# LunaJang/Metabuli_work

Measured on AMD Instinct MI355X. Metric: reads/sec classified (150bp & 10kb) vs GTDB-scale DB at 1/2/4/8 MI355X, higher is better.
Workload: dtype u64

## Files before the change

include/mtb_gpu.h:

```cpp
#ifndef MTB_GPU_H
#define MTB_GPU_H

#include <stddef.h>
#include <stdint.h>

#ifdef __cplusplus
extern "C" {
#endif

#define MTB_OK 0
#define MTB_RETRY 1
#define MTB_ERR_ARG (-1)
#define MTB_ERR_IO (-2)
#define MTB_ERR_HIP (-3)
#define MTB_ERR_DB (-4)
#define MTB_ERR_OOM (-5)
#define MTB_ERR_UNSUPPORTED (-6)
#define MTB_ERR_INTERNAL (-7)

#define MTB_INPUT_DEVICE 1u
#define MTB_KEEP_STAGES 2u
#define MTB_MATCH_ONLY 4u

typedef struct mtb_params {
// ... 77 lines not shown
                      mtb_ctx** out);
void mtb_close(mtb_ctx* ctx);
const char* mtb_last_error(void);
int mtb_set_stream(mtb_ctx* ctx, void* hip_stream);
uint64_t mtb_db_kmers(const mtb_ctx* ctx);
uint64_t mtb_workspace_bytes(const mtb_ctx* ctx);
int mtb_open_phases(const mtb_ctx* ctx, double* sec, int n);
int mtb_set_workspace_cap(mtb_ctx* ctx, uint64_t bytes);
int mtb_release_workspace(mtb_ctx* ctx);
int mtb_ctx_device(const mtb_ctx* ctx);

int mtb_classify_batch(mtb_ctx* ctx, const char* seq, const uint64_t* off, const char* seq2,
                       const uint64_t* off2, uint32_t n_reads, uint32_t flags, mtb_result* results);
int mtb_get_taxcnt(mtb_ctx* ctx, mtb_taxcnt* out, uint64_t capacity, uint64_t* n_out);
int mtb_device_results(mtb_ctx* ctx, void** results, void** taxcnt, uint64_t* n_taxcnt);
int mtb_last_counts(const mtb_ctx* ctx, uint64_t* query_kmers, uint64_t* matches);
int mtb_last_stats(const mtb_ctx* ctx, uint64_t* out, int n);
int mtb_last_stage_ms(const mtb_ctx* ctx, float* ms, int n);
int mtb_last_kernel_ms(const mtb_ctx* ctx, float* ms, int n);
int mtb_copy_results(mtb_ctx* ctx, void* dst, int dst_on_device);
int mtb_copy_taxcnt(mtb_ctx* ctx, void* dst, int dst_on_device, uint64_t* n_out);

int mtb_get_query_kmers(mtb_ctx* ctx, mtb_kmer* out, uint64_t capacity, uint64_t* n_out);
int mtb_get_matches(mtb_ctx* ctx, mtb_match* out, uint64_t capacity, uint64_t* n_out);
int mtb_assign_matches(mtb_ctx* ctx, const mtb_match* matches, uint64_t n_matches,
                       const uint32_t* query_len, uint32_t n_reads, mtb_result* results);

int mtb_mask_reads(mtb_ctx* ctx, const char* seq, const uint64_t* off, uint32_t n_reads, char* out);

int mtb_memcpy(void* dst, const void* src, uint64_t bytes);

int mtb_hamming(int device, const uint64_t* query, const uint64_t* target, uint64_t n, uint8_t* sum, uint16_t* fwd,
                uint16_t* rev);

#define MTB_PIN_SCORE_INCREMENT 0
#define MTB_PIN_HAMMING_INCREMENT 1
#define MTB_PIN_IS_CONSECUTIVE 2
#define MTB_PIN_IS_CONSECUTIVE2 3
#define MTB_PIN_MATCH_SCORE 4
#define MTB_PIN_RIGHT_PART_SCORE 5
#define MTB_PIN_LEFT_PART_SCORE 6
#define MTB_PIN_RIGHT_PART_HAMMING 7
#define MTB_PIN_LEFT_PART_HAMMING 8
#define MTB_PIN_MAX_COVERED_LENGTH 9
#define MTB_PIN_QUERY_KMER_NUMBER 10
#define MTB_PIN_TAXONOMER_SHAPE 11
// ... 150 lines not shown
```

metabuli_work_amd/_lib.py:

```python
import ctypes
import pathlib

from ._abi import MtbClassifyOpts, MtbClassifyStats, MtbDbHost, MtbDbResident, MtbEmStats, MtbParams, MtbReadBatch

_HERE = pathlib.Path(__file__).resolve().parent
LIB_PATH = _HERE / "libmtbgpu.so"
_LIB = None

EXPORTED = [
    "mtb_default_params", "mtb_load_db_parameters", "mtb_open", "mtb_open_host", "mtb_close", "mtb_last_error",
    "mtb_set_stream", "mtb_db_kmers", "mtb_classify_batch", "mtb_get_taxcnt", "mtb_device_results",
    "mtb_clone", "mtb_last_counts", "mtb_last_stats", "mtb_last_stage_ms", "mtb_last_kernel_ms", "mtb_copy_results", "mtb_get_query_kmers",
    "mtb_get_matches", "mtb_assign_matches", "mtb_build_db", "mtb_free_built", "mtb_reader_open", "mtb_reader_next",
    "mtb_reader_close", "mtb_taxon_rank", "mtb_write_classifications", "mtb_partition_bounds", "mtb_copy_matches",
    "mtb_assign_chunks", "mtb_open_resident", "mtb_write_report", "mtb_copy_taxcnt", "mtb_original_taxid",
    "mtb_taxon_lineage", "mtb_start_classify", "mtb_get_em_mappings", "mtb_em", "mtb_write_em_results",
    "mtb_ctx_device", "mtb_start_classify_multi", "mtb_mask_reads", "mtb_workspace_bytes", "mtb_set_workspace_cap",
    "mtb_open_phases", "mtb_start_classify_partitioned", "mtb_release_workspace", "mtb_hamming", "mtb_memcpy",
    "mtb_line_ext_check", "mtb_link_check", "mtb_pin_eval", "mtb_sort_pairs",
    "mtb_merge_db", "mtb_merge_db_dirs", "mtb_merge_last_ms", "mtb_merge_tile_items",
]


class MtbError(RuntimeError):
    pass


def lib() -> ctypes.CDLL:
    global _LIB
    if _LIB is not None:
        return _LIB
    if not LIB_PATH.exists():
        raise MtbError(f"{LIB_PATH} not built: the HIP extension is required (no CPU fallback)")
    L = ctypes.CDLL(str(LIB_PATH))
    vp, u32, u64, i32 = ctypes.c_void_p, ctypes.c_uint32, ctypes.c_uint64, ctypes.c_int
    P = ctypes.POINTER
    L.mtb_default_params.argtypes = [P(MtbParams)]
    L.mtb_default_params.restype = None
    L.mtb_load_db_parameters.argtypes = [ctypes.c_char_p, P(MtbParams)]
    L.mtb_open.argtypes = [ctypes.c_char_p, P(MtbParams), i32, P(vp)]
    L.mtb_open_host.argtypes = [P(MtbDbHost), P(MtbParams), i32, P(vp)]
    L.mtb_open_resident.argtypes = [P(MtbDbResident), P(MtbDbHost), P(MtbParams), i32, P(vp)]
    L.mtb_close.argtypes = [vp]
    L.mtb_clone.argtypes = [vp, P(vp)]
    L.mtb_close.restype = None
    L.mtb_last_error.restype = ctypes.c_char_p
    L.mtb_set_stream.argtypes = [vp, vp]
    L.mtb_db_kmers.argtypes = [vp]
    L.mtb_db_kmers.restype = u64
    L.mtb_workspace_bytes.argtypes = [vp]
    L.mtb_workspace_bytes.restype = u64
    L.mtb_set_workspace_cap.argtypes = [vp, u64]
    L.mtb_release_workspace.argtypes = [vp]
    L.mtb_open_phases.argtypes = [vp, P(ctypes.c_double), i32]
    L.mtb_classify_batch.argtypes = [vp, vp, vp, vp, vp, u32, u32, vp]
    L.mtb_get_taxcnt.argtypes = [vp, vp, u64, P(u64)]
    L.mtb_device_results.argtypes = [vp, P(vp), P(vp), P(u64)]
    L.mtb_last_counts.argtypes = [vp, P(u64), P(u64)]
    L.mtb_last_stats.argtypes = [vp, P(u64), i32]
    L.mtb_last_stage_ms.argtypes = [vp, P(ctypes.c_float), i32]
    L.mtb_last_kernel_ms.argtypes = [vp, P(ctypes.c_float), i32]
    L.mtb_copy_results.argtypes = [vp, vp, i32]
    L.mtb_copy_taxcnt.argtypes = [vp, vp, i32, P(u64)]
    L.mtb_get_query_kmers.argtypes = [vp, vp, u64, P(u64)]
    L.mtb_get_matches.argtypes = [vp, vp, u64, P(u64)]
    L.mtb_assign_matches.argtypes = [vp, vp, u64, vp, u32, vp]
    L.mtb_partition_bounds.argtypes = [vp, u64, u64, i32, vp, vp]
    L.mtb_copy_matches.argtypes = [vp, vp, vp, vp, i32]
    L.mtb_assign_chunks.argtypes = [vp, vp, u64, vp, u32, vp, u32, u32, vp]
    L.mtb_reader_open.argtypes = [ctypes.c_char_p, ctypes.c_char_p, P(vp)]
    L.mtb_reader_next.argtypes = [vp, u32, u64, P(MtbReadBatch)]
    L.mtb_reader_close.argtypes = [vp]
    L.mtb_reader_close.restype = None
    L.mtb_taxon_rank.argtypes = [vp, ctypes.c_int32]
    L.mtb_taxon_rank.restype = ctypes.c_char_p
    L.mtb_write_classifications.argtypes = [vp, ctypes.c_char_p, i32, P(MtbReadBatch), vp, vp, u32]
    L.mtb_original_taxid.argtypes = [vp, ctypes.c_int32]
    L.mtb_original_taxid.restype = ctypes.c_int32
    L.mtb_taxon_lineage.argtypes = [vp, ctypes.c_int32]
    L.mtb_taxon_lineage.restype = ctypes.c_char_p
    L.mtb_start_classify.argtypes = [vp, P(MtbClassifyOpts), P(MtbClassifyStats)]
    L.mtb_start_classify_multi.argtypes = [P(vp), i32, P(MtbClassifyOpts), P(MtbClassifyStats)]
    L.mtb_start_classify_partitioned.argtypes = [P(vp), i32, P(MtbClassifyOpts), P(MtbClassifyStats)]
    L.mtb_ctx_device.argtypes = [vp]
    L.mtb_mask_reads.argtypes = [vp, vp, vp, u32, vp]
    L.mtb_hamming.argtypes = [i32, vp, vp, u64, vp, vp, vp]
    L.mtb_pin_eval.argtypes = [i32, i32, vp, vp, vp, u64, vp, vp]
    L.mtb_sort_pairs.argtypes = [i32, vp, vp, u64, i32, i32, vp, vp]
# ... 22 lines not shown
```

metabuli_work_amd/csrc/mtb_api.hip:

```cpp
#include <chrono>
#include <cmath>
#include <cstdio>
#include <cstring>
#include <string>
#include <vector>
#include <algorithm>
#include <memory>
#include <charconv>
#include <mutex>
#include <unordered_map>

#include "mtb_host.h"
#include "mtb_launch.h"
#include <cstdlib>

using namespace mtb;

#define HIP_TRY(x)                                                                                   \
    do {                                                                                             \
        hipError_t e_ = (x);                                                                         \
        if (e_ != hipSuccess) {                                                                      \
            set_error(std::string("HIP error ") + hipGetErrorString(e_) + " at " #x);                 \
            return e_ == hipErrorOutOfMemory ? MTB_ERR_OOM : MTB_ERR_HIP;                            \
        }                                                                                            \
// ... 91 lines not shown
    uint64_t rankLo = 0, rankHi = ~0ull;
    int joinMode = 0;
    uint64_t* tileRec = nullptr;
    uint32_t* tilePre = nullptr;
    uint64_t nTiles = 0;
    uint32_t sweepNom = 2048;
    uint32_t sweepLdsCap = ~0u;
    bool sweepSmall = false;
    bool filterThreadMajor = false;
    int sweepPersist = 1;
    uint32_t matchWinCap = ~0u;
    bool directJoin = true;
    bool directRetry = false;
    int pruneAfter = 2;
    int bigGroups = 1;
    bool fuseFilter = true;
    bool radixDigits = true;
    bool radixAtomicFirst = false;
    int binnedSort = 0;
    uint64_t binRcForce = 0;
    bool binDigits = true;
    bool uniformUnits = true;
    uint32_t upr = 0;
    uint64_t binHost[kSortBins] = {};
    bool noFilter = false;
    uint32_t spillShift = 0;
    bool sparse = false;
    uint32_t maxW = 0;
    int sortLoFine = kQuerySortLoFine;
    bool forceGeneric = false;
    bool segsortGlobal = false;
    uint32_t mergeSeg = 0;
    int waveTaxon = -1;
    int emulateAll = 0;
    bool pruneCompact = true;
    bool noAlias = false;
    uint64_t aliasBytes = 0;
    int32_t* spOf = nullptr;
    int32_t maxTax = 0;
    int32_t *tNodeOf = nullptr, *tNodeTax = nullptr, *tParent = nullptr, *tDepth = nullptr, *tSpParent = nullptr;
    uint8_t* tFlags = nullptr;
    uint32_t cladePerMatch = 2;
    std::vector<int32_t> hNodeOf;
    std::vector<std::string> hRank;
    HostTaxonomy hTax;
    mutable std::vector<std::string> lineage;
// ... 251 lines not shown
    if (const char* e = getenv("MTB_K6_ALIAS")) c->noAlias = atoi(e) == 0;
    if (c->forceGeneric) c->matchWinCap = 0;
    c->dir = make_aa_dir(c->D, par->kmer_format);
    HIP_TRY(hipMalloc(&c->dirMem, (c->dir.R + 1) * sizeof(uint64_t)));
    c->dir.dir = c->dirMem;
    build_aa_dir(c->db, c->D, c->dir, c->dirMem, s);
    HIP_TRY(hipStreamSynchronize(s));
    c->openS[2] = since(tp);
    if (const char* e = getenv("MTB_JOIN"))
        c->joinMode = !strcmp(e, "sort") ? 1 : !strcmp(e, "probe") ? 2 : !strcmp(e, "sweep") ? 3 : 0;
    if (const char* e = getenv("MTB_SWEEP_NOM")) c->sweepNom = std::max(64u, std::min(4096u, (uint32_t)atoi(e)));
    if (const char* e = getenv("MTB_SWEEP_LDS")) c->sweepLdsCap = (uint32_t)strtoul(e, nullptr, 10);
    if (const char* e = getenv("MTB_SWEEP_PERSIST")) c->sweepPersist = std::max(0, std::min(2, atoi(e)));
    if (const char* e = getenv("MTB_SWEEP_SMALL")) c->sweepSmall = atoi(e) != 0;
    if (const char* e = getenv("MTB_FILTER_PACK")) c->filterThreadMajor = std::string(e) == "thread";
    if ((c->sweepSmall || c->sweepPersist == 2) && !getenv("MTB_SWEEP_NOM")) c->sweepNom = 1024;
    if (const char* e = getenv("MTB_FILTER")) c->noFilter = atoi(e) == 0;
    if (const char* e = getenv("MTB_RADIX_DIGITS")) c->radixDigits = atoi(e) != 0;
    if (const char* e = getenv("MTB_RADIX_ATOMIC_FIRST")) c->radixAtomicFirst = atoi(e) != 0;
    if (const char* e = getenv("MTB_K1F_BINS")) c->binnedSort = atoi(e);
    if (const char* e = getenv("MTB_K1F_BINS_RC")) c->binRcForce = strtoull(e, nullptr, 10);
    if (const char* e = getenv("MTB_K1F_BINS_DIG")) c->binDigits = atoi(e) != 0;
    if (const char* e = getenv("MTB_UNIFORM_UNITS")) c->uniformUnits = atoi(e) != 0;
    if (!c->forceGeneric && !(c->joinMode == 3 && c->noFilter)) {
        HIP_TRY(hipMalloc(&c->lines, kProbeLines * sizeof(ProbeLine)));
        HIP_TRY(hipMemsetAsync(c->lines, 0, kProbeLines * sizeof(ProbeLine), s));
        build_probe_lines(c->db, c->D, c->dir, c->lines, s);
        const char* ll = getenv("MTB_LINK_LINES");
        if ((!ll || atoi(ll) != 0) && c->joinMode != 2 && c->joinMode != 3) {
            if (hipMalloc(&c->link, kLinkSlots * sizeof(uint64_t)) == hipSuccess) {
                build_link_lines(c->lines, c->link, s);
            } else {
                (void)hipGetLastError();
                c->link = nullptr;
            }
        }
        HIP_TRY(hipStreamSynchronize(s));
        c->openS[3] = since(tp);
        const char* ri = getenv("MTB_RUN_INDEX");
        if ((!ri || atoi(ri) != 0) && c->joinMode != 3) {
            uint32_t* pop = nullptr;
            void* tmp = nullptr;
            uint64_t P = 0;
            HIP_TRY(hipMalloc(&c->lineP, (kProbeLines + 1) * sizeof(uint64_t)));
            HIP_TRY(hipMalloc(&pop, kProbeLines * sizeof(uint32_t)));
            HIP_TRY(hipMalloc(&tmp, scan_tmp_elems(kProbeLines) * sizeof(uint64_t)));
// ... 176 lines not shown
    c->matchWinCap = src->matchWinCap;
    c->directJoin = src->directJoin;
    c->directRetry = src->directRetry;
    c->pruneAfter = src->pruneAfter;
    c->bigGroups = src->bigGroups;
    c->fuseFilter = src->fuseFilter;
    c->presentShare = src->presentShare;
    c->spillShift = src->spillShift;
    c->sortLoFine = src->sortLoFine;
    c->forceGeneric = src->forceGeneric;
    c->segsortGlobal = src->segsortGlobal;
    c->mergeSeg = src->mergeSeg;
    c->waveTaxon = src->waveTaxon;
    c->emulateAll = src->emulateAll;
    c->pruneCompact = src->pruneCompact;
    c->noAlias = src->noAlias;
    c->noFilter = src->noFilter;
    c->radixDigits = src->radixDigits;
    c->radixAtomicFirst = src->radixAtomicFirst;
    c->binnedSort = src->binnedSort;
    c->binRcForce = src->binRcForce;
    c->binDigits = src->binDigits;
    c->uniformUnits = src->uniformUnits;
    bind_workspace(c, src->ws.cap);
    *out = c;
    return MTB_OK;
}

#define MTB_BATCH_BUFS(X) \
    X(seq1) X(off1) X(seq2) X(off2) X(meta) X(reserve) X(slotOff) X(qlen) X(scanTmp) X(keysA) X(valsA) X(keysB) \
    X(valsB) X(radixCounts) X(radixOffs) X(readCnt) X(mOff) X(matches) X(matchesSorted) X(segScratch) X(maxSeg) \
    X(errFlag) X(ordKA) X(ordVA) X(ordKB) X(ordVB) X(matchWin) X(unitRead) X(unitInfo) X(waveList) X(waveCount) \
    X(devStats) X(mStage) X(mRank) X(mDirect) X(ovFlag) X(mTotal) X(qFrom) X(probeStats) X(longList) X(longCnt) \
    X(qStart) X(chunkIn) X(chunkCnt) X(chunkSrcOff) X(liveCnt) X(liveOff) X(segLen) X(sizeLists) X(digA) \
    X(digB) X(binCnt) X(binTab) X(local) X(paths) X(comb) X(conn) X(spScore) X(spKeep) X(runFlag) X(runCnt) \
    X(runScan) X(pathCnt) X(gStart) X(sStart) X(runGroup) X(clade) X(tcPool) X(tcLen) X(tcOff) X(tcOut) X(results) \
    X(emMap) X(emCnt) X(emScratch) X(emPacked) X(emCnt32) X(emOff) X(maskOut1) X(maskOut2) X(maskProb) \
    X(maskScale) X(readLens) X(readCnt64)
static std::vector<DevBuf*> batch_bufs(mtb_ctx* c) {
#define MTB_BUF_PTR(n) &c->n,
    return {MTB_BATCH_BUFS(MTB_BUF_PTR)};
#undef MTB_BUF_PTR
}

static const char* const* batch_buf_names() {
#define MTB_BUF_NAME(n) #n,
// ... 325 lines not shown
            HIP_TRY(hipGetLastError());
            if (R) c->presentShare = std::max(c->presentShare, std::min(1.0, 1.125 * (double)Q / (double)R));
            bool over = false;
            for (int r = 0; r < kSortBins; r++) over |= c->binHost[r] > rc;
            if (!over) {
                binRc = rc;
                break;
            }
            c->stats[15]++;
            cap = std::min<uint64_t>(R, Q + Q / 8);
            binned = false;
        }
        for (int pass = 0; pass < 2 && !binRc; pass++) {
            HIP_TRY(c->keysB.ensure(8 * cap));
            HIP_TRY(c->valsB.ensure(4 * cap));
            if (digits) HIP_TRY(c->digA.ensure(cap));
            cap = std::min<uint64_t>(c->keysB.bytes / 8, c->valsB.bytes / 4);
            if (digits) cap = std::min<uint64_t>(cap, c->digA.bytes);
            Q = launch_extract_filter(dSeq1, dOff1, dSeq2, dOff2, c->meta.as<ReadMeta>(), c->slotOff.as<uint64_t>(),
                                      c->unitRead.as<uint32_t>(), U, C, c->tables, c->par.kmer_format, c->par.syncmer,
                                      c->par.smer_len, c->unitInfo.as<uint64_t>(), c->lines, c->keysB.as<uint64_t>(),
                                      c->valsB.as<uint32_t>(), c->mTotal.as<unsigned long long>(), c->rankLo,
                                      c->rankHi, &c->Qall, cap, c->filterThreadMajor, s,
                                      digits ? c->digA.as<uint8_t>() : nullptr, nullptr, 0, nullptr, c->upr, c->link);
            HIP_TRY(hipGetLastError());
            if (Q == ~0ull) {
                set_error("internal error: K1F sequence stage overflow");
                return MTB_ERR_INTERNAL;
            }
            if (R) c->presentShare = std::max(c->presentShare, std::min(1.0, 1.125 * (double)Q / (double)R));
            if (Q <= cap) break;
            cap = std::min<uint64_t>(R, Q + Q / 8);
            c->stats[15]++;
        }
        HIP_TRY(c->keysA.ensure(8 * std::max<uint64_t>(Q, 1)));
        HIP_TRY(c->valsA.ensure(4 * std::max<uint64_t>(Q, 1)));
        if (digits) HIP_TRY(c->digB.ensure(std::max<uint64_t>(Q, 16)));
        qk = c->keysB.as<uint64_t>();
        qi = c->valsB.as<uint32_t>();
    } else if (filt) {
        if (probe) HIP_TRY(c->qFrom.ensure(8 * Rc + 8 * kDbPad));
        Q = launch_filter(c->keysA.as<uint64_t>(), R, c->lines, c->keysB.as<uint64_t>(), c->valsB.as<uint32_t>(),
                          probe ? c->qFrom.as<uint64_t>() : nullptr, c->mTotal.as<unsigned long long>(), c->rankLo,
                          c->rankHi, &c->Qall, s);
        qk = c->keysB.as<uint64_t>();
        qi = c->valsB.as<uint32_t>();
        qf = c->qFrom.as<uint64_t>();
// ... 946 lines not shown
    }
    if (nTop > cap) return MTB_RETRY;
    uint64_t w = 0;
    for (uint32_t i = 0; i < S; i++) {
        if (!isTop[i]) continue;
        if (sp_ids) sp_ids[w] = spTax[i];
        if (sp_probs) sp_probs[w] = p[i];
        if (sp_counts) sp_counts[w] = (unsigned int)(p[i] * (double)qc);
        w++;
    }
    return MTB_OK;
}

int mtb_copy_taxcnt(mtb_ctx* c, void* dst, int dst_on_device, uint64_t* n_out) {
    if (!c || (!dst && c->nTaxcnt)) return MTB_ERR_ARG;
    if (n_out) *n_out = c->nTaxcnt;
    if (c->nTaxcnt)
        HIP_TRY(hipMemcpyAsync(dst, c->tcOut.p, sizeof(mtb_taxcnt) * c->nTaxcnt,
                               dst_on_device ? hipMemcpyDeviceToDevice : hipMemcpyDeviceToHost, c->stream));
    HIP_TRY(hipStreamSynchronize(c->stream));
    return MTB_OK;
}

int mtb_get_query_kmers(mtb_ctx* c, mtb_kmer* out, uint64_t cap, uint64_t* n_out) {
    if (!c || !n_out) return MTB_ERR_ARG;
    *n_out = c->Q;
    if (!c->keepStages) { set_error("batch was not run with MTB_KEEP_STAGES"); return MTB_ERR_ARG; }
    if (c->probed) { set_error("the probe join keeps no sorted query k-mers (MTB_JOIN=probe)"); return MTB_ERR_ARG; }
    if (!c->qSlots) { set_error("no query k-mers kept"); return MTB_ERR_ARG; }
    if (cap < c->Q) return MTB_RETRY;
    std::vector<uint64_t> k(c->Q), ui((c->unitInfo.bytes + 7) / 8);
    std::vector<uint32_t> v(c->Q);
    const void* kp = c->qKeys;
    const void* vp = c->qSlots;
    if (c->Q) {
        HIP_TRY(hipMemcpy(k.data(), kp, 8 * c->Q, hipMemcpyDeviceToHost));
        HIP_TRY(hipMemcpy(v.data(), vp, 4 * c->Q, hipMemcpyDeviceToHost));
        HIP_TRY(hipMemcpy(ui.data(), c->unitInfo.p, c->unitInfo.bytes, hipMemcpyDeviceToHost));
    }
    const bool packed = c->par.kmer_format == 2;
    for (uint64_t i = 0; i < c->Q; i++)
        out[i] = mtb_kmer{packed ? host_from_rank_form(k[i]) : k[i], slot_info(v[i], c->chunkC, ui.data(),
                                                                               c->par.kmer_format)};
    return MTB_OK;
}

// ... 209 lines not shown
```

metabuli_work_amd/csrc/mtb_kernels.hip:

```cpp
#include "mtb_launch.h"

#include <cstring>

namespace mtb {

constexpr int kBlock = 256;
constexpr int kWaves = kBlock / 64;

__device__ __forceinline__ unsigned long long wave_inclusive_scan(unsigned long long x) {
    const int lane = threadIdx.x & 63;
#pragma unroll
    for (int d = 1; d < 64; d <<= 1) {
        unsigned long long y = __shfl_up(x, d, 64);
        if (lane >= d) x += y;
    }
    return x;
}

__device__ __forceinline__ unsigned long long block_exclusive_scan(unsigned long long x, unsigned long long* total) {
    __shared__ unsigned long long wsum[kWaves];
    const int lane = threadIdx.x & 63, w = threadIdx.x >> 6;
    unsigned long long inc = wave_inclusive_scan(x);
    if (lane == 63) wsum[w] = inc;
    __syncthreads();
// ... 185 lines not shown
};

struct UnitWindows {
    const uint8_t* seq;
    int s0, e0;
    int pFirst, nWin;
    bool fromLeft, comp;
    uint64_t info0;
    uint64_t stretch;
};

__device__ __forceinline__ UnitWindows unit_windows(uint64_t u, uint64_t nUnits, uint32_t C,
                                                    const uint8_t* __restrict__ seq1, const uint64_t* __restrict__ off1,
                                                    const uint8_t* __restrict__ seq2, const uint64_t* __restrict__ off2,
                                                    const ReadMeta* __restrict__ meta, const uint64_t* __restrict__ uOff,
                                                    const uint32_t* __restrict__ unitRead, int kmerFormat,
                                                    uint32_t upr) {
    UnitWindows w{};
    if (u >= nUnits) return w;
    const uint32_t r = upr ? (uint32_t)(u / upr) : unitRead[u];
    const ReadMeta m = meta[r];
    const uint64_t first = upr ? (uint64_t)r * upr : uOff[r];
    w.stretch = first | (upr ? (uint64_t)upr : uOff[r + 1] - first) << 40;
    uint32_t local = (uint32_t)(u - first);
    const uint32_t c1 = upr ? 1u : (uint32_t)(m.w1 + C - 1) / C, c2 = upr ? 1u : (uint32_t)(m.w2 + C - 1) / C;
    uint32_t cpf = c1;
    int mate = 0;
    if (local >= 6 * c1) { local -= 6 * c1; mate = 1; cpf = c2; }
    const int frame = (int)(local / cpf);
    const int chunk = (int)(local % cpf);
    const int W = mate ? m.w2 : m.w1;
    w.pFirst = chunk * (int)C;
    w.nWin = min((int)C, W - w.pFirst);
    if (w.nWin <= 0) return w;
    w.seq = mate ? seq2 + off2[r] : seq1 + off1[r];
    const int len = mate ? m.len2 : m.len1;
    const int used = mate ? m.ql2 : m.ql1;
    const uint32_t posOffset = mate ? (uint32_t)m.ql1 + 3u : 0u;
    const bool fwd = frame < 3;
    int begin;
    if (fwd) begin = frame;
    else { begin = (len % 3) - (frame % 3); if (begin < 0) begin += 3; }
    w.s0 = begin;
    w.e0 = begin + used - 1;
    w.fromLeft = (kmerFormat == 2) ? fwd : !fwd;
    w.comp = !fwd;
    const uint32_t pos0 = w.fromLeft ? (uint32_t)(w.s0 + 3 * w.pFirst) : (uint32_t)(w.e0 - 3 * (w.pFirst + 8) + 1);
    w.info0 = pack_info(r + 1, pos0 + posOffset, (uint32_t)frame);
    return w;
}

struct WinScanner {
    const UnitWindows& w;
    const uint8_t* seq;
    const uint8_t* sBase;
    const int8_t *sAA, *sNum;
    int syncmer, nSm;
    uint64_t smMask;
    uint64_t aaAcc = 0, dnaAcc = 0, smAcc = 0;
    uint64_t sm0 = 0, sm1 = 0, sm2 = 0, sm3 = 0, sm4 = 0, sm5 = 0, sm6 = 0, sm7 = 0;
    int run = 0, j;
    uint32_t first7 = 0, firstAA = 0, lastAA = 0;

    __device__ __forceinline__ WinScanner(const UnitWindows& w_, const uint8_t* b, const int8_t* a, const int8_t* n,
                                          int sync, int smerLen, const uint8_t* seqAt)
        : w(w_), seq(seqAt), sBase(b), sAA(a), sNum(n), syncmer(sync), nSm(8 - smerLen + 1),
          smMask((smerLen >= 13) ? ~0ull : ((1ull << (5 * smerLen)) - 1)), j(w_.pFirst) {
        if (w.nWin > 0)
            for (int k = 0; k < 7; k++) codon();
    }
    __device__ __forceinline__ void codon() {
// ... 2193 lines not shown
    }
    unsigned long long tot;
    const unsigned long long off =
        block_exclusive_scan((unsigned long long)__popc(mask) | ((unsigned long long)emitted << 32), &tot) &
        0xFFFFFFFFull;
    if (threadIdx.x == 0) {
        const unsigned long long present = tot & 0xFFFFFFFFull;
        sBase = present ? atomicAdd(counter, present) : 0;
        if (tot >> 32) atomicAdd(counter + 1, tot >> 32);
    }
    __syncthreads();
    uint64_t pos = sBase + off;
#pragma unroll
    for (int j = 0; j < kFilterPer; j++) {
        if (!((mask >> j) & 1u)) continue;
        qkey[pos] = k[j];
        qslot[pos] = (uint32_t)(base + 256ull * j);
        if (FROM) qfrom[pos] = line_lower_bound(lines, k[j] >> 24);
        pos++;
    }
}

constexpr uint32_t kBinStage = 2560;
constexpr uint32_t kSeqStage = 10240;
template <int kPer, bool kJMajor, bool kBinned = false, int kLink = 0, bool kSplit = false, bool kSeqLds = false,
          bool kWavePack = false>
__global__ void __launch_bounds__(256) __attribute__((amdgpu_waves_per_eu(kLink == 4 ? 4 : 1))) k_extract_filter(const uint8_t* __restrict__ seq1, const uint64_t* __restrict__ off1,
                                                        const uint8_t* __restrict__ seq2, const uint64_t* __restrict__ off2,
                                                        const ReadMeta* __restrict__ meta, const uint64_t* __restrict__ uOff,
                                                        const uint32_t* __restrict__ unitRead, uint64_t nUnits, uint32_t C,
                                                        ExtractTables tabs, int kmerFormat, int syncmer, int smerLen,
                                                        uint64_t* __restrict__ unitInfo, const ProbeLine* __restrict__ lines,
                                                        uint64_t* __restrict__ qkey, uint32_t* __restrict__ qslot,
                                                        unsigned long long* __restrict__ counter, uint64_t rankLo,
                                                        uint64_t rankHi, uint64_t cap, uint8_t* __restrict__ qdig,
                                                        unsigned long long* __restrict__ binCnt, uint64_t binRc,
                                                        uint32_t upr, const uint64_t* __restrict__ link,
                                                        int emitPerBlock = 0) {
    static_assert(kLink == 0 || kPer % 2 == 0, "windows probed in pairs");
    __shared__ uint8_t sBase[256];
    __shared__ uint32_t sBin[256];
    __shared__ uint32_t sBinBase[256];
    extern __shared__ uint64_t sStageKey[];
    __shared__ int8_t sAA[64], sNum[64];
    __shared__ unsigned long long sOut;
    __shared__ uint32_t sMaxWin, sCnt[kPer * kWaves], sEx[kWaves][64];
    const int lane = (int)(threadIdx.x & 63), wv = (int)(threadIdx.x >> 6);
    const unsigned long long ltMask = (1ull << lane) - 1;
    if (threadIdx.x == 0) sMaxWin = 0;
    load_extract_tables(tabs, sBase, sAA, sNum);
    const uint64_t u = (uint64_t)blockIdx.x * blockDim.x + threadIdx.x;
    const uint64_t slotBase = (u >> 6) * 64ull * C + (u & 63u);
    const UnitWindows w = unit_windows(u, nUnits, C, seq1, off1, seq2, off2, meta, uOff, unitRead, kmerFormat, upr);
    if (w.nWin > 0) {
        reinterpret_cast<ulonglong2*>(unitInfo)[u] = make_ulonglong2(w.info0, w.stretch);
        atomicMax(&sMaxWin, (uint32_t)w.nWin);
    }
    __shared__ uint8_t sSeq[kSeqLds ? kSeqStage : 1];
    const uint8_t* seqAt = kSeqLds ? sSeq : w.seq;
    if constexpr (kSeqLds) {
        const uint64_t u0 = (uint64_t)blockIdx.x * blockDim.x, uL = min(u0 + blockDim.x, nUnits) - 1;
        const uint64_t r0 = u0 / upr, r1 = uL / upr;
        const uint64_t a1 = off1[r0], n1 = off1[r1 + 1] - a1;
        const uint64_t a2 = seq2 ? off2[r0] : 0, n2 = seq2 ? off2[r1 + 1] - a2 : 0;
        if (n1 + n2 <= kSeqStage) {
            for (uint32_t i = threadIdx.x; i < n1; i += blockDim.x) sSeq[i] = seq1[a1 + i];
            for (uint32_t i = threadIdx.x; i < n2; i += blockDim.x) sSeq[n1 + i] = seq2[a2 + i];
            if (w.nWin > 0) {
                const uint64_t r = u / upr;
                seqAt = (u - r * upr) >= 6u ? sSeq + n1 + (off2[r] - a2) : sSeq + (off1[r] - a1);
            }
        } else if (threadIdx.x == 0) {
            atomicOr(counter + 1, 1ull << 63);
        }
    }
    __syncthreads();
    WinScanner sc(w, sBase, sAA, sNum, syncmer, smerLen, seqAt);
    __syncthreads();
    const uint32_t gEnd = min(C, sMaxWin);
    uint32_t emitted = 0;
    for (uint32_t g = 0; g < gEnd; g += kPer) {
        const uint32_t* const src = kLink ? reinterpret_cast<const uint32_t*>(link) : reinterpret_cast<const uint32_t*>(lines);
        uint64_t k[kPer];
        uint32_t word[kPer], sh[kPer];
        uint32_t f0 = 0, t0 = 0, h0 = 0, y0 = 0;
        bool ok0 = false;
#pragma unroll
        for (int j = 0; j < kPer; j++) {
            k[j] = (int)(g + j) < w.nWin ? sc.next() : kSentinel;
            if constexpr (kLink) {
                const uint64_t r = k[j] >> 24;
                const bool ok = k[j] != kSentinel && r >= rankLo && r < rankHi;
                const uint32_t h = sc.first7, y = sc.lastAA, f = sc.firstAA;
                if (!(j & 1)) {
                    f0 = f, h0 = h, y0 = y, ok0 = ok;
                    t0 = (uint32_t)(r - (uint64_t)f * kLinkSlots);
                    continue;
                }
                const bool shared = ok0 && ok && t0 == h;
                word[j - 1] = !ok0 ? 0u : (shared ? 2u * t0 + 1u : 2u * h0);
                word[j] = !ok ? 0u : 2u * h;
                sh[j - 1] = !ok0 ? 32u : (shared ? f0 : y0);
                sh[j] = !ok ? 32u : y;
                if constexpr (!kSplit) {
                    word[j - 1] = src[word[j - 1]];
                    word[j] = src[word[j]];
                }
            } else {
                word[j] = 0;
                sh[j] = 32;
                const uint64_t xr = k[j] >> 24;
                if (k[j] != kSentinel && xr >= rankLo && xr < rankHi) {
// ... 146 lines not shown
    for (int d = 32; d > 0; d >>= 1) emitted += (uint32_t)__shfl_xor((int)emitted, d, 64);
    if (emitPerBlock) {
        __shared__ uint32_t sEmit[kWaves];
        if ((threadIdx.x & 63) == 0) sEmit[wv] = emitted;
        __syncthreads();
        if (threadIdx.x == 0) {
            uint32_t e = 0;
#pragma unroll
            for (int i = 0; i < kWaves; i++) e += sEmit[i];
            if (e) atomicAdd(counter + 1, (unsigned long long)e);
        }
        return;
    }
    if ((threadIdx.x & 63) == 0 && emitted) atomicAdd(counter + 1, (unsigned long long)emitted);
}

uint64_t launch_extract_filter(const uint8_t* seq1, const uint64_t* off1, const uint8_t* seq2, const uint64_t* off2,
                               const ReadMeta* meta, const uint64_t* uOff, const uint32_t* unitRead, uint64_t nUnits,
                               uint32_t C, const HostTables& t, int kmerFormat, int syncmer, int smerLen,
                               uint64_t* unitInfo, const ProbeLine* lines, uint64_t* qkey, uint32_t* qslot,
                               unsigned long long* counter, uint64_t rankLo, uint64_t rankHi, uint64_t* emitted,
                               uint64_t cap, bool threadMajor, hipStream_t s, uint8_t* qdig,
                               unsigned long long* binCnt, uint64_t binRc, uint64_t* binHost, uint32_t upr,
                               const uint64_t* link) {
    if (binRc) {
        threadMajor = false;
        hipMemsetAsync(binCnt, 0, kSortBins * sizeof(unsigned long long), s);
    }
    hipMemsetAsync(counter, 0, 2 * sizeof(unsigned long long), s);
    if (nUnits) {
        const uint64_t threads = (nUnits + 63) / 64 * 64;
        static const int per = getenv("MTB_FILTER_PER") && atoi(getenv("MTB_FILTER_PER")) == 8 ? 8 : 16;
        const bool jMajor = !threadMajor;
        const unsigned blocks = (unsigned)((threads + 255) / 256);
        const size_t lds = binRc ? kBinStage * (sizeof(uint64_t) + sizeof(uint32_t)) : 0;
#define MTB_EF(P, J)                                                                                                  \
    k_extract_filter<P, J, false, 0, true><<<blocks, 256, lds, s>>>(seq1, off1, seq2, off2, meta, uOff, unitRead, nUnits, C, \
                                                  extract_tables(t), kmerFormat, syncmer, smerLen, unitInfo, lines, qkey, \
                                                  qslot, counter, rankLo, rankHi, cap, qdig, binCnt, binRc, upr, nullptr)
        if (binRc) {
            k_extract_filter<kFilterPer, true, true><<<blocks, 256, lds, s>>>(
                seq1, off1, seq2, off2, meta, uOff, unitRead, nUnits, C, extract_tables(t), kmerFormat, syncmer, smerLen,
                unitInfo, lines, qkey, qslot, counter, rankLo, rankHi, cap, qdig, binCnt, binRc, upr, nullptr);
        } else if (link && jMajor) {
            const char* lf = getenv("MTB_LINK_FORM");
            const std::string f = lf ? lf : "w4i";
#define MTB_EFL(P, W, S)                                                                                            \
    k_extract_filter<P, true, false, W, S><<<blocks, 256, lds, s>>>(                                                \
        seq1, off1, seq2, off2, meta, uOff, unitRead, nUnits, C, extract_tables(t), kmerFormat, syncmer, smerLen,   \
        unitInfo, lines, qkey, qslot, counter, rankLo, rankHi, cap, qdig, binCnt, binRc, upr, link)
            const char* eb = getenv("MTB_K1F_EMIT_BLOCK");
            const int emitBlock = !eb || atoi(eb) != 0;
#define MTB_EFLS(P, W, S)                                                                                           \
    k_extract_filter<P, true, false, W, S, true><<<blocks, 256, lds, s>>>(                                          \
        seq1, off1, seq2, off2, meta, uOff, unitRead, nUnits, C, extract_tables(t), kmerFormat, syncmer, smerLen,   \
        unitInfo, lines, qkey, qslot, counter, rankLo, rankHi, cap, qdig, binCnt, binRc, upr, link, emitBlock)
            const char* wp = getenv("MTB_K1F_WAVEPACK");
            const bool wavePack = wp && atoi(wp) != 0;
            const char* sl = getenv("MTB_K1F_SEQ_LDS");
            const bool seqLds = upr && (!sl || atoi(sl) != 0);
            if (seqLds && wavePack && f == "w4i")
                k_extract_filter<16, true, false, 4, false, true, true><<<blocks, 256, lds, s>>>(
                    seq1, off1, seq2, off2, meta, uOff, unitRead, nUnits, C, extract_tables(t), kmerFormat, syncmer,
                    smerLen, unitInfo, lines, qkey, qslot, counter, rankLo, rankHi, cap, qdig, binCnt, binRc, upr, link);
            else if (seqLds && f == "w3i") MTB_EFLS(16, 3, false);
            else if (seqLds && f == "w3i8") MTB_EFLS(8, 3, false);
            else if (seqLds) MTB_EFLS(16, 4, false);
            else if (f == "w3i") MTB_EFL(16, 3, false);
            else if (f == "w3s") MTB_EFL(16, 3, true);
            else if (f == "w4s") MTB_EFL(16, 4, true);
            else if (f == "w3i8") MTB_EFL(8, 3, false);
            else if (f == "w3s8") MTB_EFL(8, 3, true);
            else MTB_EFL(16, 4, false);
#undef MTB_EFLS
#undef MTB_EFL
        } else if (per == 8) {
            if (jMajor) MTB_EF(8, true);
            else MTB_EF(8, false);
        } else {
            if (jMajor) MTB_EF(kFilterPer, true);
            else MTB_EF(kFilterPer, false);
        }
#undef MTB_EF
// ... 936 lines not shown
```

metabuli_work_amd/csrc/mtb_launch.h:

```cpp
#pragma once
#include <hip/hip_runtime.h>
#include <stdint.h>

#include <utility>

#include "mtb_device.h"

namespace mtb {

constexpr int kErrTaxid = 1;
constexpr int kErrStagedRead = 2;
constexpr int kErrProbeStash = 3;
constexpr int kErrProbeCount = 4;
constexpr int kErrRunOutsideDb = 5;
constexpr int kErrLiveCount = 6;

struct ReadMeta {
    int32_t len1, len2, ql1, ql2, w1, w2;
};

struct HostTables {
    uint8_t base[256];
    int8_t aa[64];
    int8_t num[64];
};

struct TaxDevice {
    const int32_t* nodeOf;
    const int32_t* nodeTax;
    const int32_t* parent;
    const int32_t* depth;
    const uint8_t* flags;
    const int32_t* spParent;
    int32_t maxTax;
};

struct AssignArgs {
    int kmerFormat, dnaShift, maxCodonShift, denominator, minConsCnt, minConsCntEuk, accessionLevel;
    float minScore, minSpScore, tieRatio;
    int generic;
    int waveTaxon = -1;
    int emulateAll = 0;
// ... 105 lines not shown
                       uint16_t* runOff, hipStream_t s);
constexpr uint32_t kExtRanks = 256;
struct alignas(64) ProbeExt {
    uint32_t w[kExtRanks / 16];
};
static_assert(sizeof(ProbeExt) == 64, "one run-length line per probe line");
void build_line_ext(const ProbeLine* lines, const uint64_t* lineP, const uint16_t* runOff, ProbeExt* ext,
                    hipStream_t s);
void launch_line_ext_check(const ProbeLine* lines, const uint64_t* lineP, const uint16_t* runOff, const ProbeExt* ext,
                           unsigned long long* out, hipStream_t s);

constexpr uint64_t kLinkSlots = 1801088541ull;
static_assert(kLinkSlots * 21 == kAARankEnd, "21^8 AA ranks");
void build_link_lines(const ProbeLine* lines, uint64_t* link, hipStream_t s);
void launch_link_check(const ProbeLine* lines, const uint64_t* link, unsigned long long* out, hipStream_t s);

uint64_t launch_extract_filter(const uint8_t* seq1, const uint64_t* off1, const uint8_t* seq2, const uint64_t* off2,
                               const ReadMeta* meta, const uint64_t* uOff, const uint32_t* unitRead, uint64_t nUnits,
                               uint32_t C, const HostTables& t, int kmerFormat, int syncmer, int smerLen,
                               uint64_t* unitInfo, const ProbeLine* lines, uint64_t* qkey, uint32_t* qslot,
                               unsigned long long* counter, uint64_t rankLo, uint64_t rankHi, uint64_t* emitted,
                               uint64_t cap, bool threadMajor, hipStream_t s,
                               uint8_t* qdig = nullptr, unsigned long long* binCnt = nullptr, uint64_t binRc = 0,
                               uint64_t* binHost = nullptr, uint32_t upr = 0, const uint64_t* link = nullptr);
uint64_t launch_filter(const uint64_t* keys, uint64_t R, const ProbeLine* lines, uint64_t* qkey, uint32_t* qslot,
                       uint64_t* qfrom, unsigned long long* counter, uint64_t rankLo, uint64_t rankHi,
                       uint64_t* emitted, hipStream_t s);
void launch_probe(const uint64_t* qkey, const uint32_t* qslot, const uint64_t* qfrom, uint64_t Q,
                  const uint64_t* unitInfo, uint32_t C, const DbRec* db, uint64_t D,
                  const int32_t* spOf, uint32_t maxTax, int kmerFormat, uint32_t* readCnt, unsigned long long* total,
                  mtb_match* buf, uint32_t* bufRank, uint64_t region, int* err, unsigned long long* stats,
                  hipStream_t s);

constexpr uint32_t kSegMaxTax = (1u << 24) - 1;
struct SegMatch {
    uint32_t posFrame, targetHam, speciesReh, dnaReh;
};
static_assert(sizeof(SegMatch) == 16, "16-B segment matches");
__host__ __device__ inline SegMatch seg_pack(const mtb_match& m) {
    return SegMatch{(uint32_t)m.qinfo | (uint32_t)(m.qinfo >> 61) << 29, m.target_id | (uint32_t)m.hamming << 24,
                    m.species_id | (uint32_t)(m.right_end_hamming & 0xFFu) << 24,
                    (m.dna_encoding & 0xFFFFFFu) | (uint32_t)(m.right_end_hamming >> 8) << 24};
}
__host__ __device__ inline mtb_match seg_expand(const SegMatch& s, uint64_t seqBits) {
    mtb_match m;
    m.qinfo = (uint64_t)(s.posFrame >> 29) << 61 | seqBits | (s.posFrame & 0x1FFFFFFFu);
    m.target_id = s.targetHam & 0xFFFFFFu;
// ... 135 lines not shown
```

Measured before the change: 34.49 million.

## Stage per-unit sequence byte ranges in LDS for long reads too

The extract-filter kernel's LDS sequence staging was limited to uniform units-per-read batches and copied each read's whole span. It now finds distinct read pointers per block with a ballot and scan, merges each unit's byte range with atomics, and copies only the needed bytes into a larger LDS buffer. Unit-to-frame ordering is also changed to frame-major interleaving, so adjacent units share a read and overlap in bases. This enables staging for long (10kb) reads by default, meant to cut redundant global reads, at the cost of extra syncs, atomics, LDS pressure and a fallback flag when ranges don't fit.

```diff
diff --git a/include/mtb_gpu.h b/include/mtb_gpu.h
--- a/include/mtb_gpu.h
+++ b/include/mtb_gpu.h
@@ -123,6 +123,8 @@
 int mtb_copy_taxcnt(mtb_ctx* ctx, void* dst, int dst_on_device, uint64_t* n_out);
 
 int mtb_get_query_kmers(mtb_ctx* ctx, mtb_kmer* out, uint64_t capacity, uint64_t* n_out);
+int mtb_unit_info(int len1, int len2, uint32_t chunk, int kmer_format, uint32_t read, uint32_t local, uint32_t p,
+                  uint64_t* info, int* n_win);
 int mtb_get_matches(mtb_ctx* ctx, mtb_match* out, uint64_t capacity, uint64_t* n_out);
 int mtb_assign_matches(mtb_ctx* ctx, const mtb_match* matches, uint64_t n_matches,
                        const uint32_t* query_len, uint32_t n_reads, mtb_result* results);
diff --git a/metabuli_work_amd/_lib.py b/metabuli_work_amd/_lib.py
--- a/metabuli_work_amd/_lib.py
+++ b/metabuli_work_amd/_lib.py
@@ -18,7 +18,7 @@
     "mtb_ctx_device", "mtb_start_classify_multi", "mtb_mask_reads", "mtb_workspace_bytes", "mtb_set_workspace_cap",
     "mtb_open_phases", "mtb_start_classify_partitioned", "mtb_release_workspace", "mtb_hamming", "mtb_memcpy",
     "mtb_line_ext_check", "mtb_link_check", "mtb_pin_eval", "mtb_sort_pairs",
-    "mtb_merge_db", "mtb_merge_db_dirs", "mtb_merge_last_ms", "mtb_merge_tile_items",
+    "mtb_merge_db", "mtb_merge_db_dirs", "mtb_merge_last_ms", "mtb_merge_tile_items", "mtb_unit_info",
 ]
 
 
@@ -64,6 +64,7 @@
     L.mtb_copy_taxcnt.argtypes = [vp, vp, i32, P(u64)]
     L.mtb_get_query_kmers.argtypes = [vp, vp, u64, P(u64)]
     L.mtb_get_matches.argtypes = [vp, vp, u64, P(u64)]
+    L.mtb_unit_info.argtypes = [i32, i32, u32, i32, u32, u32, u32, P(u64), P(i32)]
     L.mtb_assign_matches.argtypes = [vp, vp, u64, vp, u32, vp]
     L.mtb_partition_bounds.argtypes = [vp, u64, u64, i32, vp, vp]
     L.mtb_copy_matches.argtypes = [vp, vp, vp, vp, i32]
diff --git a/metabuli_work_amd/csrc/mtb_api.hip b/metabuli_work_amd/csrc/mtb_api.hip
--- a/metabuli_work_amd/csrc/mtb_api.hip
+++ b/metabuli_work_amd/csrc/mtb_api.hip
@@ -137,6 +137,7 @@
     bool binDigits = true;
     bool uniformUnits = true;
     uint32_t upr = 0;
+    bool longFast = true;
     uint64_t binHost[kSortBins] = {};
     bool noFilter = false;
     uint32_t spillShift = 0;
@@ -434,6 +435,7 @@
     if (const char* e = getenv("MTB_K1F_BINS_RC")) c->binRcForce = strtoull(e, nullptr, 10);
     if (const char* e = getenv("MTB_K1F_BINS_DIG")) c->binDigits = atoi(e) != 0;
     if (const char* e = getenv("MTB_UNIFORM_UNITS")) c->uniformUnits = atoi(e) != 0;
+    if (const char* e = getenv("MTB_LONG_FAST")) c->longFast = atoi(e) != 0;
     if (!c->forceGeneric && !(c->joinMode == 3 && c->noFilter)) {
         HIP_TRY(hipMalloc(&c->lines, kProbeLines * sizeof(ProbeLine)));
         HIP_TRY(hipMemsetAsync(c->lines, 0, kProbeLines * sizeof(ProbeLine), s));
@@ -656,6 +658,7 @@
     c->binRcForce = src->binRcForce;
     c->binDigits = src->binDigits;
     c->uniformUnits = src->uniformUnits;
+    c->longFast = src->longFast;
     bind_workspace(c, src->ws.cap);
     *out = c;
     return MTB_OK;
@@ -1027,7 +1030,8 @@
                                       c->par.smer_len, c->unitInfo.as<uint64_t>(), c->lines, c->keysB.as<uint64_t>(),
                                       c->valsB.as<uint32_t>(), c->mTotal.as<unsigned long long>(), c->rankLo,
                                       c->rankHi, &c->Qall, cap, c->filterThreadMajor, s,
-                                      digits ? c->digA.as<uint8_t>() : nullptr, nullptr, 0, nullptr, c->upr, c->link);
+                                      digits ? c->digA.as<uint8_t>() : nullptr, nullptr, 0, nullptr, c->upr, c->link,
+                                      c->longFast);
             HIP_TRY(hipGetLastError());
             if (Q == ~0ull) {
                 set_error("internal error: K1F sequence stage overflow");
@@ -2020,6 +2024,19 @@
     return MTB_OK;
 }
 
+int mtb_unit_info(int len1, int len2, uint32_t chunk, int kmer_format, uint32_t read, uint32_t local, uint32_t p,
+                  uint64_t* info, int* n_win) {
+    if (!info || !n_win || chunk == 0 || len1 < 0 || len2 < 0) return MTB_ERR_ARG;
+    const ReadMeta m = read_meta_of_lens(len1, len2);
+    if (m.w1 < 1 || (len2 && m.w2 < 1)) { *n_win = 0; *info = 0; return MTB_OK; }
+    const uint32_t units = 6u * ((uint32_t)(m.w1 + chunk - 1) / chunk + (uint32_t)(m.w2 + chunk - 1) / chunk);
+    if (local >= units) return MTB_ERR_ARG;
+    const UnitGeom g = unit_geom(m, local, chunk, 0, kmer_format);
+    *n_win = g.nWin;
+    *info = (int)p < g.nWin ? unit_info_at(pack_info(read + 1, g.pos0, (uint32_t)g.frame), p, kmer_format) : 0;
+    return MTB_OK;
+}
+
 int mtb_get_query_kmers(mtb_ctx* c, mtb_kmer* out, uint64_t cap, uint64_t* n_out) {
     if (!c || !n_out) return MTB_ERR_ARG;
     *n_out = c->Q;
diff --git a/metabuli_work_amd/csrc/mtb_kernels.hip b/metabuli_work_amd/csrc/mtb_kernels.hip
--- a/metabuli_work_amd/csrc/mtb_kernels.hip
+++ b/metabuli_work_amd/csrc/mtb_kernels.hip
@@ -231,31 +231,16 @@
     const ReadMeta m = meta[r];
     const uint64_t first = upr ? (uint64_t)r * upr : uOff[r];
     w.stretch = first | (upr ? (uint64_t)upr : uOff[r + 1] - first) << 40;
-    uint32_t local = (uint32_t)(u - first);
-    const uint32_t c1 = upr ? 1u : (uint32_t)(m.w1 + C - 1) / C, c2 = upr ? 1u : (uint32_t)(m.w2 + C - 1) / C;
-    uint32_t cpf = c1;
-    int mate = 0;
-    if (local >= 6 * c1) { local -= 6 * c1; mate = 1; cpf = c2; }
-    const int frame = (int)(local / cpf);
-    const int chunk = (int)(local % cpf);
-    const int W = mate ? m.w2 : m.w1;
-    w.pFirst = chunk * (int)C;
-    w.nWin = min((int)C, W - w.pFirst);
+    const UnitGeom g = unit_geom(m, (uint32_t)(u - first), C, upr, kmerFormat);
+    w.pFirst = g.pFirst;
+    w.nWin = g.nWin;
     if (w.nWin <= 0) return w;
-    w.seq = mate ? seq2 + off2[r] : seq1 + off1[r];
-    const int len = mate ? m.len2 : m.len1;
-    const int used = mate ? m.ql2 : m.ql1;
-    const uint32_t posOffset = mate ? (uint32_t)m.ql1 + 3u : 0u;
-    const bool fwd = frame < 3;
-    int begin;
-    if (fwd) begin = frame;
-    else { begin = (len % 3) - (frame % 3); if (begin < 0) begin += 3; }
-    w.s0 = begin;
-    w.e0 = begin + used - 1;
-    w.fromLeft = (kmerFormat == 2) ? fwd : !fwd;
-    w.comp = !fwd;
-    const uint32_t pos0 = w.fromLeft ? (uint32_t)(w.s0 + 3 * w.pFirst) : (uint32_t)(w.e0 - 3 * (w.pFirst + 8) + 1);
-    w.info0 = pack_info(r + 1, pos0 + posOffset, (uint32_t)frame);
+    w.seq = g.mate ? seq2 + off2[r] : seq1 + off1[r];
+    w.s0 = g.s0;
+    w.e0 = g.e0;
+    w.fromLeft = g.fromLeft;
+    w.comp = g.frame >= 3;
+    w.info0 = pack_info(r + 1, g.pos0, (uint32_t)g.frame);
     return w;
 }
 
@@ -2495,7 +2480,12 @@
 }
 
 constexpr uint32_t kBinStage = 2560;
-constexpr uint32_t kSeqStage = 10240;
+constexpr uint32_t kSeqRanges = 2 + (256 - 2) / 6;
+constexpr uint32_t kSeqGroups = (256 + 20) / 6;
+constexpr uint32_t kSeqStage = 12288;
+static_assert(3 * (64 * (kSeqGroups + 2) + 7 * kSeqRanges) + 2 * kSeqRanges <= kSeqStage,
+              "a block's bases fit the LDS stage");
+typedef const uint8_t __attribute__((address_space(1)))* GlobalBytes;
 template <int kPer, bool kJMajor, bool kBinned = false, int kLink = 0, bool kSplit = false, bool kSeqLds = false,
           bool kWavePack = false>
 __global__ void __launch_bounds__(256) __attribute__((amdgpu_waves_per_eu(kLink == 4 ? 4 : 1))) k_extract_filter(const uint8_t* __restrict__ seq1, const uint64_t* __restrict__ off1,
@@ -2521,34 +2511,77 @@
     const int lane = (int)(threadIdx.x & 63), wv = (int)(threadIdx.x >> 6);
     const unsigned long long ltMask = (1ull << lane) - 1;
     if (threadIdx.x == 0) sMaxWin = 0;
-    load_extract_tables(tabs, sBase, sAA, sNum);
     const uint64_t u = (uint64_t)blockIdx.x * blockDim.x + threadIdx.x;
     const uint64_t slotBase = (u >> 6) * 64ull * C + (u & 63u);
     const UnitWindows w = unit_windows(u, nUnits, C, seq1, off1, seq2, off2, meta, uOff, unitRead, kmerFormat, upr);
-    if (w.nWin > 0) {
+    __shared__ uint8_t sSeq[kSeqLds ? kSeqStage : 1];
+    __shared__ const uint8_t* sRngSeq[kSeqLds ? kSeqRanges : 1];
+    __shared__ uint32_t sRngLo[kSeqLds ? kSeqRanges : 1], sRngHi[kSeqLds ? kSeqRanges : 1];
+    __shared__ const uint8_t* sWaveLastSeq[kWaves];
+    __shared__ uint32_t sWaveHeads[kWaves];
+    const bool hasWin = w.nWin > 0;
+    const uint32_t nb3 = hasWin ? 3u * (uint32_t)(w.nWin + 7) : 0u;
+    const uint32_t bLo = !hasWin ? 0u : w.fromLeft ? (uint32_t)(w.s0 + 3 * w.pFirst) : (uint32_t)(w.e0 - 3 * w.pFirst + 1) - nb3;
+    const uint32_t bHi = bLo + nb3;
+    if constexpr (kSeqLds) {
+        if (lane == 63) sWaveLastSeq[wv] = w.seq;
+        if (threadIdx.x < kSeqRanges) { sRngLo[threadIdx.x] = ~0u; sRngHi[threadIdx.x] = 0u; }
+    }
+    load_extract_tables(tabs, sBase, sAA, sNum);
+    if (hasWin) {
         reinterpret_cast<ulonglong2*>(unitInfo)[u] = make_ulonglong2(w.info0, w.stretch);
         atomicMax(&sMaxWin, (uint32_t)w.nWin);
     }
-    __shared__ uint8_t sSeq[kSeqLds ? kSeqStage : 1];
     const uint8_t* seqAt = kSeqLds ? sSeq : w.seq;
+    UnitWindows ws = w;
     if constexpr (kSeqLds) {
-        const uint64_t u0 = (uint64_t)blockIdx.x * blockDim.x, uL = min(u0 + blockDim.x, nUnits) - 1;
-        const uint64_t r0 = u0 / upr, r1 = uL / upr;
-        const uint64_t a1 = off1[r0], n1 = off1[r1 + 1] - a1;
-        const uint64_t a2 = seq2 ? off2[r0] : 0, n2 = seq2 ? off2[r1 + 1] - a2 : 0;
-        if (n1 + n2 <= kSeqStage) {
-            for (uint32_t i = threadIdx.x; i < n1; i += blockDim.x) sSeq[i] = seq1[a1 + i];
-            for (uint32_t i = threadIdx.x; i < n2; i += blockDim.x) sSeq[n1 + i] = seq2[a2 + i];
-            if (w.nWin > 0) {
-                const uint64_t r = u / upr;
-                seqAt = (u - r * upr) >= 6u ? sSeq + n1 + (off2[r] - a2) : sSeq + (off1[r] - a1);
+        const uint8_t* prevSeq = (const uint8_t*)__shfl_up((unsigned long long)w.seq, 1, 64);
+        if (lane == 0) prevSeq = wv ? sWaveLastSeq[wv - 1] : nullptr;
+        const bool head = hasWin && prevSeq != w.seq;
+        const unsigned long long hb = __ballot(head);
+        if (lane == 0) sWaveHeads[wv] = (uint32_t)__popcll(hb);
+        __syncthreads();
+        uint32_t rng = (uint32_t)__popcll(hb & (ltMask | (1ull << lane))), nRng = 0;
+#pragma unroll
+        for (int i = 0; i < kWaves; i++) {
+            rng += i < wv ? sWaveHeads[i] : 0u;
+            nRng += sWaveHeads[i];
+        }
+        rng -= 1;
+        const bool rngOk = nRng <= kSeqRanges;
+        if (hasWin && rngOk) {
+            atomicMin(&sRngLo[rng], bLo);
+            atomicMax(&sRngHi[rng], bHi);
+            if (head) sRngSeq[rng] = w.seq;
+        }
+        __syncthreads();
+        static_assert(kSeqRanges <= 64, "one range per lane");
+        const uint32_t myLo = (uint32_t)lane < nRng && rngOk ? sRngLo[lane] : 0u;
+        const uint32_t myLen = (uint32_t)lane < nRng && rngOk ? sRngHi[lane] - myLo : 0u;
+        const uint32_t inc = (uint32_t)wave_inclusive_scan((unsigned long long)myLen);
+        const uint32_t total = (uint32_t)__shfl((int)inc, 63, 64);
+        const bool fits = rngOk && total <= kSeqStage;
+        if (fits) {
+            for (uint32_t r = 0; r < nRng; r++) {
+                const uint32_t at = (uint32_t)__shfl((int)(inc - myLen), (int)r, 64);
+                const uint32_t len = (uint32_t)__shfl((int)myLen, (int)r, 64);
+                const GlobalBytes src = (GlobalBytes)(sRngSeq[r] + (uint32_t)__shfl((int)myLo, (int)r, 64));
+                for (uint32_t i = threadIdx.x; i < len; i += blockDim.x) sSeq[at + i] = src[i];
             }
         } else if (threadIdx.x == 0) {
             atomicOr(counter + 1, 1ull << 63);
         }
+        const uint32_t rl = hasWin && fits ? rng : 0u;
+        const uint32_t at = (uint32_t)__shfl((int)(inc - myLen), (int)rl, 64);
+        const uint32_t lo = (uint32_t)__shfl((int)myLo, (int)rl, 64);
+        if (!fits) ws.nWin = 0;
+        seqAt = sSeq + (hasWin && fits ? at : 0u);
+        ws.pFirst = 0;
+        ws.s0 = (int)(bLo - lo);
+        ws.e0 = (int)(bHi - lo) - 1;
     }
     __syncthreads();
-    WinScanner sc(w, sBase, sAA, sNum, syncmer, smerLen, seqAt);
+    WinScanner sc(ws, sBase, sAA, sNum, syncmer, smerLen, seqAt);
     __syncthreads();
     const uint32_t gEnd = min(C, sMaxWin);
     uint32_t emitted = 0;
@@ -2560,7 +2593,7 @@
         bool ok0 = false;
 #pragma unroll
         for (int j = 0; j < kPer; j++) {
-            k[j] = (int)(g + j) < w.nWin ? sc.next() : kSentinel;
+            k[j] = (int)(g + j) < ws.nWin ? sc.next() : kSentinel;
             if constexpr (kLink) {
                 const uint64_t r = k[j] >> 24;
                 const bool ok = k[j] != kSentinel && r >= rankLo && r < rankHi;
@@ -2753,7 +2786,7 @@
                                unsigned long long* counter, uint64_t rankLo, uint64_t rankHi, uint64_t* emitted,
                                uint64_t cap, bool threadMajor, hipStream_t s, uint8_t* qdig,
                                unsigned long long* binCnt, uint64_t binRc, uint64_t* binHost, uint32_t upr,
-                               const uint64_t* link) {
+                               const uint64_t* link, bool stageAll) {
     if (binRc) {
         threadMajor = false;
         hipMemsetAsync(binCnt, 0, kSortBins * sizeof(unsigned long long), s);
@@ -2789,7 +2822,7 @@
             const char* wp = getenv("MTB_K1F_WAVEPACK");
             const bool wavePack = wp && atoi(wp) != 0;
             const char* sl = getenv("MTB_K1F_SEQ_LDS");
-            const bool seqLds = upr && (!sl || atoi(sl) != 0);
+            const bool seqLds = (upr || stageAll) && (!sl || atoi(sl) != 0);
             if (seqLds && wavePack && f == "w4i")
                 k_extract_filter<16, true, false, 4, false, true, true><<<blocks, 256, lds, s>>>(
                     seq1, off1, seq2, off2, meta, uOff, unitRead, nUnits, C, extract_tables(t), kmerFormat, syncmer,
diff --git a/metabuli_work_amd/csrc/mtb_launch.h b/metabuli_work_amd/csrc/mtb_launch.h
--- a/metabuli_work_amd/csrc/mtb_launch.h
+++ b/metabuli_work_amd/csrc/mtb_launch.h
@@ -18,6 +18,52 @@
 struct ReadMeta {
     int32_t len1, len2, ql1, ql2, w1, w2;
 };
+
+struct UnitGeom {
+    int mate, frame;
+    int pFirst, nWin;
+    int s0, e0;
+    bool fromLeft;
+    uint32_t pos0;
+};
+
+__host__ __device__ inline UnitGeom unit_geom(const ReadMeta& m, uint32_t local, uint32_t C, uint32_t upr,
+                                              int kmerFormat) {
+    UnitGeom g{};
+    const uint32_t c1 = upr ? 1u : (uint32_t)(m.w1 + C - 1) / C, c2 = upr ? 1u : (uint32_t)(m.w2 + C - 1) / C;
+    uint32_t cpf = c1;
+    if (local >= 6 * c1) { local -= 6 * c1; g.mate = 1; cpf = c2; }
+    const uint32_t grp = local / 6u;
+    g.frame = (int)(local - 6u * grp);
+    const bool fwd = g.frame < 3;
+    g.fromLeft = (kmerFormat == 2) ? fwd : !fwd;
+    const int chunk = g.fromLeft ? (int)grp : (int)cpf - 1 - (int)grp;
+    const int W = g.mate ? m.w2 : m.w1;
+    g.pFirst = chunk * (int)C;
+    g.nWin = W - g.pFirst < (int)C ? W - g.pFirst : (int)C;
+    if (g.nWin <= 0) return g;
+    const int len = g.mate ? m.len2 : m.len1;
+    const int used = g.mate ? m.ql2 : m.ql1;
+    const uint32_t posOffset = g.mate ? (uint32_t)m.ql1 + 3u : 0u;
+    int begin;
+    if (fwd) begin = g.frame;
+    else { begin = (len % 3) - (g.frame % 3); if (begin < 0) begin += 3; }
+    g.s0 = begin;
+    g.e0 = begin + used - 1;
+    g.pos0 = (g.fromLeft ? (uint32_t)(g.s0 + 3 * g.pFirst) : (uint32_t)(g.e0 - 3 * (g.pFirst + 8) + 1)) + posOffset;
+    return g;
+}
+
+__host__ __device__ inline ReadMeta read_meta_of_lens(int len1, int len2) {
+    ReadMeta m;
+    m.len1 = len1; m.len2 = len2;
+    m.ql1 = max_covered_length(len1);
+    m.ql2 = len2 ? max_covered_length(len2) : 0;
+    m.w1 = query_kmer_number(len1) / 6;
+    m.w2 = len2 ? query_kmer_number(len2) / 6 : 0;
+    if (m.w2 < 0) m.w2 = 0;
+    return m;
+}
 
 struct HostTables {
     uint8_t base[256];
@@ -169,7 +215,8 @@
                                unsigned long long* counter, uint64_t rankLo, uint64_t rankHi, uint64_t* emitted,
                                uint64_t cap, bool threadMajor, hipStream_t s,
                                uint8_t* qdig = nullptr, unsigned long long* binCnt = nullptr, uint64_t binRc = 0,
-                               uint64_t* binHost = nullptr, uint32_t upr = 0, const uint64_t* link = nullptr);
+                               uint64_t* binHost = nullptr, uint32_t upr = 0, const uint64_t* link = nullptr,
+                               bool stageAll = false);
 uint64_t launch_filter(const uint64_t* keys, uint64_t R, const ProbeLine* lines, uint64_t* qkey, uint32_t* qslot,
                        uint64_t* qfrom, unsigned long long* counter, uint64_t rankLo, uint64_t rankHi,
                        uint64_t* emitted, hipStream_t s);
```

After: 34.15 million. 0.99x the previous value.
